# VisualComputingInstitute/diffusion-e2e-ft

Measured on AMD Instinct MI355X. Metric: images/sec (768x768, 1-step UNet fwd) full path: VAE encode + SD-v2 UNet @t=999 + VAE decode, higher is better.
Workload: dtype f16

## Files before the change

### diffusion-e2e-ft_amd/_lib.py

```python
import ctypes as C
import os

import torch

from . import build as _build

_LIB = None

F32, F16, BF16 = 0, 1, 2
_DT = {torch.float32: F32, torch.float16: F16, torch.bfloat16: BF16}


def dtype_id(dt):
    try:
        return _DT[dt]
    except KeyError:
        raise TypeError("libe2eft supports float32/float16/bfloat16, got %s" % dt)


class ConvDesc(C.Structure):
    _fields_ = [(n, C.c_int32) for n in (
        "dtype", "batch", "hin", "win", "hl", "wl", "c1", "ldx1", "c2", "ldx2", "kh", "kw", "stride", "pad_t", "pad_l",
        "hout", "wout", "cout", "ldo", "ldr", "ldw")] + [("alpha", C.c_float)]

# ... 47 lines not shown
class NormalGtDesc(C.Structure):
    _fields_ = [(n, C.c_int32) for n in ("batch", "height", "width", "raw_dtype")]


NORMAL_GT_U8, NORMAL_GT_F32 = range(2)


class DsineRgbDesc(C.Structure):
    _fields_ = [(n, C.c_int32) for n in ("batch", "height", "width", "out_layout")]


class DiffusionDesc(C.Structure):
    _fields_ = [(n, C.c_int32) for n in ("dtype", "dtype_out", "prediction", "rows", "hw", "c", "batch", "ldx0", "ldn", "ldy", "n_timesteps")]


DIFFUSION_ADD_NOISE, DIFFUSION_VELOCITY = range(2)
PREDICTION_TYPES = {"epsilon": 0, "v_prediction": 1}


RGB_HWC, RGB_CHW = range(2)
DSINE_RGB_WS_INTS = 6


OPT_PERSISTENT, OPT_PERSISTENT_GRID, OPT_NARROW_CONV, OPT_NARROW_MFMA, OPT_IGEMM_GENERAL_OPERANDS, OPT_IGEMM2_WAVES, OPT_PATCH_CONV, OPT_THIN_INPUT_CONV, OPT_FUSED_NORM, OPT_ATTN_DMA, OPT_UPCONV_PHASES, OPT_PATCH_CONV_2X2, OPT_PERSISTENT_MIN_QROUNDS, OPT_GN_APPLY_ITERS, OPT_F32_SPLIT, OPT_F32_SPLIT_ATTN, OPT_PATCH_MFMA = range(17)

_P = C.c_void_p
_I = C.c_int32
_L = C.c_int64
_F = C.c_float
_Z = C.c_size_t

SIGNATURES = {
    "e2eft_version": (_I, []),
    "e2eft_last_error": (C.c_char_p, []),
    "e2eft_build_id": (C.c_char_p, []),
    "e2eft_set_option": (_I, [_I, _I]),
    "e2eft_get_option": (_I, [_I]),
    "e2eft_conv2d_fwd": (_I, [C.POINTER(ConvDesc), _P, _P, _P, _P, _P, _P, _P, _P]),
    "e2eft_gemm": (_I, [C.POINTER(GemmDesc), _P, _P, _P, _P, _P, _P]),
    "e2eft_conv2d_fwd_gnstats": (_I, [C.POINTER(ConvDesc), _P, _P, _P, _P, _P, _P, _P, _P, _Z, C.POINTER(C.c_int32), _P]),
    "e2eft_conv2d_splitk_workspace_bytes": (_Z, [C.POINTER(ConvDesc)]),
    "e2eft_conv2d_fwd_splitk": (_I, [C.POINTER(ConvDesc), _P, _P, _P, _P, _P, _P, _P, _P, _Z, _P]),
    "e2eft_gemm_gnstats": (_I, [C.POINTER(GemmDesc), _P, _P, _P, _P, _P, _I, _P, _Z, C.POINTER(C.c_int32), _P]),
    "e2eft_groupnorm_fwd_pre": (_I, [C.POINTER(GroupNormDesc), _P, _P, _P, _P, _P, _P, _I, _P, _I, _P, _Z, _P]),
    "e2eft_groupnorm_coeff_offset": (_Z, [C.POINTER(GroupNormDesc)]),
    "e2eft_groupnorm_fwd_stats": (_I, [C.POINTER(GroupNormDesc), _P, _P, _P, _P, _I, _P, _I, _P, _Z, _P]),
    "e2eft_conv2d_fwd_normed_supported": (_I, [C.POINTER(ConvDesc)]),
    "e2eft_upconv2x_fwd_supported": (_I, [C.POINTER(ConvDesc)]),
    "e2eft_upconv2x_fwd": (_I, [C.POINTER(ConvDesc), _P, _P, _P, _P, _P, _Z, C.POINTER(C.c_int32), _P]),
    "e2eft_groupnorm_fwd_split": (_I, [C.POINTER(GroupNormDesc), _P, _P, _P, _P, _I, _P, _P, _I, _P, _Z, _P]),
    "e2eft_f32_split_weight": (_I, [_P, _L, _I, _P, _P, _P]),
    "e2eft_f32_split2_cat": (_I, [_P, _I, _I, _P, _I, _I, _L, _P, _I, _P, _P]),
    "e2eft_f32_split2": (_I, [_P, _L, _I, _I, _P, _I, _P, _P]),
    "e2eft_f32_split2_cols": (_I, [_P, _I, _I, _P, _I, _I, _L, _P, _I, _P, _P]),
    "e2eft_f32_split_wgrad_finish": (_I, [_P, _P, _P, _L, _I, _I, _P, _P, _P, _P]),
    "e2eft_conv2d_fwd_f32split_supported": (_I, [C.POINTER(ConvDesc)]),
    "e2eft_conv2d_fwd_f32split": (_I, [C.POINTER(ConvDesc), _P, _P, _P, _P, _P, _P, _P, _P, _Z, C.POINTER(C.c_int32), _P]),
    "e2eft_upconv2x_fwd_f32split_supported": (_I, [C.POINTER(ConvDesc)]),
    "e2eft_upconv2x_fwd_f32split": (_I, [C.POINTER(ConvDesc), _P, _P, _P, _P, _P, _P, _P, _Z, C.POINTER(C.c_int32), _P]),
    "e2eft_gemm_f32split_supported": (_I, [C.POINTER(GemmDesc)]),
    "e2eft_attn_f32split_supported": (_I, [C.POINTER(AttnDesc), _I]),
    "e2eft_gemm_f32split": (_I, [C.POINTER(GemmDesc), _P, _P, _P, _P, _P, _P, _P, _P]),
    "e2eft_conv2d_fwd_normed": (_I, [C.POINTER(ConvDesc), _P, _P, _P, _I, _P, _P, _P, _P, _P, _P, _Z, C.POINTER(C.c_int32), _P]),
    "e2eft_groupnorm_workspace_bytes": (_Z, [C.POINTER(GroupNormDesc)]),
    "e2eft_groupnorm_fwd": (_I, [C.POINTER(GroupNormDesc), _P, _P, _P, _P, _P, _P, _Z, _P]),
    "e2eft_layernorm_fwd": (_I, [_I, _L, _I, _I, _I, _F, _P, _P, _P, _P, _P]),
    "e2eft_geglu_fwd": (_I, [_I, _L, _I, _I, _I, _P, _P, _P]),
    "e2eft_softmax_rows": (_I, [_I, _L, _I, _L, _F, _P, _P]),
    "e2eft_softmax_rows_causal": (_I, [_I, _L, _I, _L, _F, _I, _P, _P]),
    "e2eft_attn_fwd": (_I, [C.POINTER(AttnDesc), _P, _P, _P, _P, _P]),
    "e2eft_attn_fwd_lse": (_I, [C.POINTER(AttnDesc), _P, _P, _P, _P, _P, _P]),
    "e2eft_attn512_workspace_bytes": (_Z, [C.POINTER(AttnDesc)]),
    "e2eft_attn512_fwd": (_I, [C.POINTER(AttnDesc), _P, _P, _P, _P, _P, _Z, _P]),
    "e2eft_attn_bwd_workspace_bytes": (_Z, [C.POINTER(AttnDesc)]),
    "e2eft_attn_bwd": (_I, [C.POINTER(AttnDesc), _P, _P, _P, _P, _P, _I, _P, _P, _I, _P, _I, _P, _I, _P, _Z, _P]),
    "e2eft_nchw_to_nhwc": (_I, [_I, _I, _I, _I, _I, _I, _I, _F, _F, _P, _P, _P]),
    "e2eft_nhwc_to_nchw": (_I, [_I, _I, _I, _I, _I, _I, _F, _F, _P, _P, _P]),
    "e2eft_copy_scale": (_I, [_I, _L, _I, _I, _I, _F, _F, _P, _P, _P]),
    "e2eft_add": (_I, [_I, _L, _I, _I, _I, _I, _P, _P, _P, _P]),
    "e2eft_timestep_embedding": (_I, [_I, _I, _I, _P, _P, _P]),
    "e2eft_silu": (_I, [_I, _L, _P, _P, _P]),
    "e2eft_depth_head": (_I, [_I, _I, _L, _I, _I, _P, _P, _P]),
    "e2eft_normal_head": (_I, [_I, _I, _I, _I, _I, _I, _F, _P, _P, _P]),
    "e2eft_ssi_loss_workspace_bytes": (_Z, [_I]),
    "e2eft_ssi_loss_fwd": (_I, [_I, _I, _P, _P, _P, _P, _P, _P, _Z, _P]),
    "e2eft_angular_loss_workspace_bytes": (_Z, [_I]),
    "e2eft_angular_loss_fwd": (_I, [_I, _I, _P, _P, _P, _P, _P, _Z, _P]),
    "e2eft_conv2d_dgrad": (_I, [C.POINTER(ConvDesc), _P, _I, _I, _P, _I, _P, _I, _P]),
    "e2eft_conv2d_wgrad_workspace_bytes": (_Z, [C.POINTER(ConvDesc), _I]),
# ... 138 lines not shown
```

### diffusion-e2e-ft_amd/csrc/api.hip

```cpp
#include "common.h"
#include <atomic>

namespace e2eft {

static thread_local char g_err[512] = "";

char* err_buf() { return g_err; }

int fail(int code, const char* fmt, ...) {
    va_list ap;
    va_start(ap, fmt);
    vsnprintf(g_err, sizeof(g_err), fmt, ap);
    va_end(ap);
    return code;
}

int check_launch(const char* what) {
    hipError_t e = hipGetLastError();
    if (e != hipSuccess) return fail(E2EFT_ERR_LAUNCH, "%s: launch failed: %s", what, hipGetErrorString(e));
    return E2EFT_OK;
}

static std::atomic<int> g_cus_of_device[64];
int device_cus() {
    int dev = 0;
    if (hipGetDevice(&dev) != hipSuccess || dev < 0 || dev >= 64) return 0;
    int n = g_cus_of_device[dev].load(std::memory_order_relaxed);
    if (n == 0) {
        if (hipDeviceGetAttribute(&n, hipDeviceAttributeMultiprocessorCount, dev) != hipSuccess || n < 8) return 0;
        n &= ~7;
        g_cus_of_device[dev].store(n, std::memory_order_relaxed);
    }
    return n;
}

static thread_local char g_tag[96] = "";
void tag_kernel(const char* fmt, ...) {
    va_list ap;
    va_start(ap, fmt);
    vsnprintf(g_tag, sizeof(g_tag), fmt, ap);
    va_end(ap);
}
const char* last_tag() { return g_tag; }

static std::atomic<int> g_opt[E2EFT_OPT_COUNT] = {{1}, {0}, {1}, {1}, {0}, {0}, {1}, {1}, {1}, {1}, {1}, {1}, {2}, {0}, {1}, {0}, {0}};

int option(int key) { return g_opt[key].load(std::memory_order_relaxed); }

}

extern "C" int e2eft_set_option(int32_t key, int32_t value) {
    using namespace e2eft;
    E2EFT_REQUIRE(key >= 0 && key < E2EFT_OPT_COUNT, "set_option: unknown key %d", key);
    bool ok = value == 0 || value == 1;
    if (key == E2EFT_OPT_PERSISTENT_GRID) ok = value == 0 || (value >= 8 && value % 8 == 0 && value <= 4096);
    if (key == E2EFT_OPT_IGEMM2_WAVES) ok = value == 0 || value == 4 || value == 8;
    if (key == E2EFT_OPT_PERSISTENT_MIN_QROUNDS) ok = value >= 1 && value <= 64;
    if (key == E2EFT_OPT_GN_APPLY_ITERS) ok = value >= 0 && value <= 16;
    if (key == E2EFT_OPT_PATCH_MFMA) ok = value >= 0 && value <= 2;
    E2EFT_REQUIRE(ok, "set_option: value %d out of range for key %d", value, key);
    g_opt[key].store(value, std::memory_order_relaxed);
    return E2EFT_OK;
}
extern "C" int e2eft_get_option(int32_t key) { return key >= 0 && key < E2EFT_OPT_COUNT ? e2eft::option(key) : -1; }

extern "C" const char* e2eft_debug_last_kernel(void) { return e2eft::last_tag(); }

extern "C" int e2eft_version(void) { return E2EFT_VERSION; }
// ... 7 lines not shown
```

### diffusion-e2e-ft_amd/csrc/gfx950.h

```cpp
#pragma once
#include "common.h"
#include <type_traits>

namespace e2eft {

template <int V> using IConst = std::integral_constant<int, V>;

template <typename T> struct Mma32x32x16;
template <> struct Mma32x32x16<f16> {
    __device__ static __forceinline__ floatx16 run(const u32x4& a, const u32x4& b, floatx16 c) {
        return __builtin_amdgcn_mfma_f32_32x32x16_f16(__builtin_bit_cast(half8, a), __builtin_bit_cast(half8, b), c, 0, 0, 0);
    }
};
template <> struct Mma32x32x16<bf16> {
    __device__ static __forceinline__ floatx16 run(const u32x4& a, const u32x4& b, floatx16 c) {
        return __builtin_amdgcn_mfma_f32_32x32x16_bf16(__builtin_bit_cast(bhalf8, a), __builtin_bit_cast(bhalf8, b), c, 0, 0, 0);
    }
};

template <typename T> struct Mma16x16x32;
template <> struct Mma16x16x32<f16> {
    __device__ static __forceinline__ floatx4 run(const u32x4& a, const u32x4& b, floatx4 c) {
        return __builtin_amdgcn_mfma_f32_16x16x32_f16(__builtin_bit_cast(half8, a), __builtin_bit_cast(half8, b), c, 0, 0, 0);
    }
};
template <> struct Mma16x16x32<bf16> {
    __device__ static __forceinline__ floatx4 run(const u32x4& a, const u32x4& b, floatx4 c) {
        return __builtin_amdgcn_mfma_f32_16x16x32_bf16(__builtin_bit_cast(bhalf8, a), __builtin_bit_cast(bhalf8, b), c, 0, 0, 0);
    }
};

typedef float float2v __attribute__((ext_vector_type(2)));
typedef __bf16 bhalf2v __attribute__((ext_vector_type(2)));
template <typename T> __device__ __forceinline__ uint32_t pack2(float lo, float hi);
template <> __device__ __forceinline__ uint32_t pack2<f16>(float lo, float hi) {
    const float2v f = {lo, hi};
    return __builtin_bit_cast(uint32_t, __builtin_convertvector(f, half2v));
}
template <> __device__ __forceinline__ uint32_t pack2<bf16>(float lo, float hi) {
    const float2v f = {lo, hi};
    return __builtin_bit_cast(uint32_t, __builtin_convertvector(f, bhalf2v));
}

__device__ __forceinline__ int fast_div(int n, int d) {
    int q = (int)((float)n * __builtin_amdgcn_rcpf((float)d));
    const int r = n - q * d;
    if (r < 0) --q;
    else if (r >= d) ++q;
    return q;
}

typedef __attribute__((address_space(3))) void* lds_ptr_t;

__device__ __forceinline__ u32x2 lds_read_tr16(const char* p) {
    typedef short short4v __attribute__((ext_vector_type(4)));
    return __builtin_bit_cast(u32x2, __builtin_amdgcn_ds_read_tr16_b64_v4i16((__attribute__((address_space(3))) short4v*)p));
}

constexpr unsigned int SRD_RECORDS = 0xE0000000u;
constexpr unsigned int SRD_OOB = 0xF0000000u;
constexpr long SRD_SPAN_MAX = 0xD0000000L, SRD_TILE_MAX = 0x40000000L;
__device__ __forceinline__ __amdgpu_buffer_rsrc_t whole_range_rsrc(const void* base) {
    return __builtin_amdgcn_make_buffer_rsrc((void*)base, 0, SRD_RECORDS, 0x00020000);
}
// ... 25 lines not shown
```

### diffusion-e2e-ft_amd/csrc/narrow.hip

```cpp
#include "gfx950.h"

namespace e2eft {

constexpr int NR_T = 16;
constexpr int NR_H = NR_T + 2;
constexpr int NR_CH = 64;
constexpr int NR_PIX = NR_CH * 2 + 16;
constexpr int NR_CO = 4;

typedef _Float16 h2 __attribute__((ext_vector_type(2)));
typedef __bf16 b2 __attribute__((ext_vector_type(2)));
typedef short s2 __attribute__((ext_vector_type(2)));

template <typename T> __device__ __forceinline__ float dot2(unsigned a, unsigned b, float c);
template <> __device__ __forceinline__ float dot2<f16>(unsigned a, unsigned b, float c) {
    return __builtin_amdgcn_fdot2(__builtin_bit_cast(h2, a), __builtin_bit_cast(h2, b), c, false);
}
template <> __device__ __forceinline__ float dot2<bf16>(unsigned a, unsigned b, float c) {
    return __builtin_amdgcn_fdot2_f32_bf16(__builtin_bit_cast(s2, a), __builtin_bit_cast(s2, b), c, false);
}
template <typename T> __device__ __forceinline__ float dot16(const u32x4& a, const u32x4& b, float s) {
    if constexpr (sizeof(T) == 4) {
        const floatx4 fa = __builtin_bit_cast(floatx4, a), fb = __builtin_bit_cast(floatx4, b);
        s = fmaf(fa[0], fb[0], s); s = fmaf(fa[1], fb[1], s); s = fmaf(fa[2], fb[2], s); s = fmaf(fa[3], fb[3], s);
    } else {
        s = dot2<T>(a[0], b[0], s); s = dot2<T>(a[1], b[1], s); s = dot2<T>(a[2], b[2], s); s = dot2<T>(a[3], b[3], s);
    }
    return s;
}

struct NarrowParams {
    const void* x;
    const void* w;
    const void* bias;
    void* out;
    int H, W, cin, ldx, ldw, cout, ldo, tiles_x, tiles_y;
    float alpha;
    const float* nrm_ad;
    const void* nrm_beta;
    int nrm_silu;
};

typedef const __attribute__((address_space(4))) u32x4* cptr_t;

template <typename T, int CO>
__global__ __launch_bounds__(256) void conv3x3_narrow_kernel(const NarrowParams p, const T* __restrict__ wg) {
    __shared__ __attribute__((aligned(16))) char halo[NR_H * NR_H * NR_PIX];
    const int tid = threadIdx.x;
    const int tx = tid & 15, ty = tid >> 4;
    const int tile = blockIdx.x;
    const int oy0 = (tile / p.tiles_x) * NR_T, ox0 = (tile % p.tiles_x) * NR_T;
    const T* xb = (const T*)p.x + (long)blockIdx.y * p.H * p.W * p.ldx;
// ... 205 lines not shown
```

### diffusion-e2e-ft_amd/csrc/norm.hip

```cpp
#include "common.h"

namespace e2eft {

struct Triple {
    float n, mean, m2;
};
__device__ __forceinline__ Triple merge(const Triple& A, const Triple& B) {
    if (B.n == 0.f) return A;
    if (A.n == 0.f) return B;
    Triple r;
    r.n = A.n + B.n;
    const float delta = B.mean - A.mean;
    const float f = B.n / r.n;
    r.mean = A.mean + delta * f;
    r.m2 = A.m2 + B.m2 + delta * delta * A.n * f;
    return r;
}

struct GnGeom {
    int batch, hw, c1, ldx1, c2, ldx2, C;
    int nchunks, cpb, nchb, pl;
    int nslabs, slab;
};

// ... 562 lines not shown
    const float mean = wave_sum(sum) / (float)c;
    float sq = 0.f;
#pragma unroll
    for (int i = 0; i < MAXI; ++i) {
        const int ch = lane + 64 * i;
        if (ch < nchunks) {
#pragma unroll
            for (int e = 0; e < EPC; ++e) { const float dd = v[i][e] - mean; sq += dd * dd; }
        }
    }
    const float rstd = rsqrtf(wave_sum(sq) / (float)c + eps);
#pragma unroll
    for (int i = 0; i < MAXI; ++i) {
        const int ch = lane + 64 * i;
        if (ch < nchunks) {
            Vec16<T> ga = ld16(gamma + ch * EPC), be = ld16(beta + ch * EPC), o;
#pragma unroll
            for (int e = 0; e < EPC; ++e) o.e[e] = from_f<T>((v[i][e] - mean) * rstd * to_f(ga.e[e]) + to_f(be.e[e]));
            st16(y + row * ldy + ch * EPC, o);
        }
    }
}

template <typename T>
__global__ __launch_bounds__(256) void softmax_rows_kernel(int ntot, long lds, float scale, T* __restrict__ s, int causal_nq) {
    constexpr int EPC = 16 / (int)sizeof(T);
    __shared__ float red[8];
    T* row = s + (long)blockIdx.x * lds;
    const int tid = threadIdx.x, lane = tid & 63, wave = tid >> 6;
    const int n = causal_nq > 0 ? min(ntot, (int)(blockIdx.x % (unsigned)causal_nq) + 1) : ntot;
    const int nfull = n / EPC;
    const float sc = scale * 1.4426950408889634f;
    float mx = -INFINITY;
    for (int ch = tid; ch < nfull; ch += 256) {
        Vec16<T> v = ld16(row + ch * EPC);
#pragma unroll
        for (int e = 0; e < EPC; ++e) mx = fmaxf(mx, to_f(v.e[e]));
    }
    for (int j = nfull * EPC + tid; j < n; j += 256) mx = fmaxf(mx, to_f(row[j]));
    mx = wave_max(mx);
    if (lane == 0) red[wave] = mx;
    __syncthreads();
    mx = fmaxf(fmaxf(red[0], red[1]), fmaxf(red[2], red[3]));
    const float mb = mx * sc;
    float sum = 0.f;
    for (int ch = tid; ch < nfull; ch += 256) {
// ... 258 lines not shown
}

extern "C" int e2eft_layernorm_fwd(int32_t dtype, int64_t rows, int32_t c, int32_t ldx, int32_t ldy, float eps,
                                   const void* x, const void* gamma, const void* beta, void* y, void* stream) {
    E2EFT_REQUIRE(x && gamma && beta && y, "layernorm: null pointer");
    E2EFT_REQUIRE(dtype >= 0 && dtype <= 2, "layernorm: bad dtype");
    const int epc = 16 / (int)dtype_size(dtype);
    E2EFT_REQUIRE(rows > 0 && c > 0 && c % epc == 0 && ldx >= c && ldy >= c && ldx % epc == 0 && ldy % epc == 0, "layernorm: shape c=%d ldx=%d ldy=%d", c, ldx, ldy);
    const int nchunks = c / epc;
    E2EFT_REQUIRE(nchunks <= 64 * 8, "layernorm: c=%d too large", c);
    const long nblk = (rows + 3) / 4;
    E2EFT_REQUIRE(nblk < 2147483647L, "layernorm: too many rows");
    hipStream_t s = (hipStream_t)stream;
    const int iters = (nchunks + 63) / 64;
#define LN_LAUNCH(T, MAXI) hipLaunchKernelGGL((layernorm_kernel<T, MAXI>), dim3((unsigned)nblk), dim3(256), 0, s, (long)rows, c, ldx, ldy, eps, (const T*)x, (const T*)gamma, (const T*)beta, (T*)y)
    E2EFT_DISPATCH_DTYPE(dtype, T, {
        if (iters <= 1) LN_LAUNCH(T, 1);
        else if (iters <= 2) LN_LAUNCH(T, 2);
        else if (iters <= 4) LN_LAUNCH(T, 4);
        else LN_LAUNCH(T, 8);
    });
#undef LN_LAUNCH
    return check_launch("layernorm");
}

extern "C" int e2eft_softmax_rows(int32_t dtype, int64_t rows, int32_t n, int64_t lds, float scale, void* sbuf, void* stream) {
    E2EFT_REQUIRE(sbuf, "softmax: null pointer");
    E2EFT_REQUIRE(dtype >= 0 && dtype <= 2, "softmax: bad dtype");
    const int epc = 16 / (int)dtype_size(dtype);
    E2EFT_REQUIRE(rows > 0 && rows < 2147483647L && n > 0 && lds >= (n + epc - 1) / epc * epc && lds % epc == 0, "softmax: shape n=%d lds=%ld", n, (long)lds);
    E2EFT_REQUIRE(scale > 0.f, "softmax: scale must be positive");
    hipStream_t s = (hipStream_t)stream;
    E2EFT_DISPATCH_DTYPE(dtype, T, hipLaunchKernelGGL((softmax_rows_kernel<T>), dim3((unsigned)rows), dim3(256), 0, s, n, (long)lds, scale, (T*)sbuf, 0));
    return check_launch("softmax_rows");
}

extern "C" int e2eft_softmax_rows_causal(int32_t dtype, int64_t rows, int32_t n, int64_t lds, float scale, int32_t nq, void* sbuf, void* stream) {
    E2EFT_REQUIRE(sbuf, "softmax_causal: null pointer");
    E2EFT_REQUIRE(dtype >= 0 && dtype <= 2, "softmax_causal: bad dtype");
    const int epc = 16 / (int)dtype_size(dtype);
    E2EFT_REQUIRE(rows > 0 && rows < 2147483647L && n > 0 && lds >= (n + epc - 1) / epc * epc && lds % epc == 0, "softmax_causal: shape n=%d lds=%ld", n, (long)lds);
    E2EFT_REQUIRE(nq > 0 && nq <= n && rows % nq == 0, "softmax_causal: nq=%d must divide rows and be <= n (self-attention)", nq);
    E2EFT_REQUIRE(scale > 0.f, "softmax_causal: scale must be positive");
    hipStream_t s = (hipStream_t)stream;
    E2EFT_DISPATCH_DTYPE(dtype, T, hipLaunchKernelGGL((softmax_rows_kernel<T>), dim3((unsigned)rows), dim3(256), 0, s, n, (long)lds, scale, (T*)sbuf, (int)nq));
    return check_launch("softmax_rows_causal");
// ... 119 lines not shown
```

### diffusion-e2e-ft_amd/modules.py

```python

import torch
from torch import nn

from . import ops
from . import autograd as F


_cached = F.cached


def packed_conv_weight(conv):
    return F.packed_conv_weight(conv, conv.weight.dtype)


def conv_nhwc(conv, x, x2=None, up_to=None, rowadd=None, residual=None, alpha=1.0, pad=None, out=None, gn_stats=True, norm=None):
    assert out is None
    return F.conv(conv, x, x2=x2, up_to=up_to, rowadd=rowadd, residual=residual, alpha=alpha, pad=pad, gn_stats=gn_stats, norm=norm)


def checkpointed(enabled, fn, *args):
    if enabled and torch.is_grad_enabled() and any(isinstance(a, torch.Tensor) and a.requires_grad for a in args):
        from torch.utils.checkpoint import checkpoint
        return checkpoint(fn, *args, use_reentrant=False)
    return fn(*args)
# ... 177 lines not shown
    def __init__(self, query_dim, heads, cross_attention_dim=None, bias=False, joint=False):
        super().__init__()
        self.heads = heads
        self.scale = (query_dim // heads) ** -0.5
        self.joint = joint
        kv = cross_attention_dim or query_dim
        self.to_q = Linear(query_dim, query_dim, bias=bias)
        self.to_k = Linear(kv, query_dim, bias=bias)
        self.to_v = Linear(kv, query_dim, bias=bias)
        self.to_out = nn.ModuleList([Linear(query_dim, query_dim), nn.Dropout(0.0)])

    def forward(self, x, ctx=None, residual=None):
        B, N, C = x.shape
        d = C // self.heads
        out = self.to_out[0]
        kv_pre = None
        shared_src = None
        if isinstance(ctx, CtxCond):
            kv_pre = ctx.kv.get(id(self))
            shared_src = ctx.src if ctx.shared else None
            ctx = ctx.ctx
        if F.needs_grad(x, ctx, self.to_q.weight, self.to_k.weight, self.to_v.weight, out.weight):
            return out(self._forward_train(x, ctx), residual=residual)
        if (CROSS_ATTN_FOLD and shared_src is not None and shared_src.shape[1] == 2 and not self.joint and self.to_q.bias is None and self.to_k.bias is None
                and self.to_v.bias is None and self.heads <= 64):
            return self._folded(x, shared_src, residual)
        fused = F.fused_attention_ok(x.dtype, d)
        dt = x.dtype
        if fused:
            if ctx is None:
                qkv = F.linear(x, (self.to_q.weight, self.to_k.weight, self.to_v.weight), owner=self, name="wqkv")
                q, k, v = qkv[..., :C], qkv[..., C:2 * C], qkv[..., 2 * C:]
            else:
                q = self.to_q(x)
                kv = kv_pre
                if kv is None or torch.is_grad_enabled():
                    kv = F.linear(ctx, (self.to_k.weight, self.to_v.weight), owner=self, name="wkv")
                k, v = kv[..., :C], kv[..., C:]
            a = ops.attention(q, k, v, self.heads, self.scale, kv_nseg=2 if self.joint else 1, kv_bmod=B // 2 if self.joint else B)
        else:
            src = x if ctx is None else ctx
            cw = lambda lin: F._cat_weight(lin, "w", (lin.weight,), dt, lin.weight.shape[1])
            a = attention_unfused(x, src, cw(self.to_q), F._vec(self.to_q.bias, dt), cw(self.to_k), F._vec(self.to_k.bias, dt), cw(self.to_v),
                                  F._vec(self.to_v.bias, dt), self.heads, self.scale, joint=self.joint)
        return out(a, residual=residual)

    def _fold(self, src, dt):
        out = self.to_out[0]
        ws = [w for w in (self.to_q.weight, self.to_k.weight, self.to_v.weight, out.weight, out.bias) if w is not None]
        key = (src.data_ptr(), src._version, tuple(src.shape), str(src.device), dt, F._key(*ws))
        hit = self.__dict__.get("_fold_cache")
        if hit is not None and hit[0] == key:
            return hit[1]
        with torch.no_grad():
            h, C = self.heads, self.to_q.weight.shape[0]
            d = C // h
            f32 = lambda w: w.detach().float().contiguous()
            wq, wk, wv, wo = f32(self.to_q.weight), f32(self.to_k.weight), f32(self.to_v.weight), f32(out.weight)
            c32 = f32(src[0])
            k = ops.gemm(c32, wk)
            v = ops.gemm(c32, wv)
            ar = torch.arange(h, device=k.device)
            Mk = torch.zeros((h, h, d), dtype=torch.float32, device=k.device)
            Mv = torch.zeros((h, h, d), dtype=torch.float32, device=k.device)
            Mk[ar, ar] = (k[0] - k[1]).view(h, d) * self.scale
            Mv[ar, ar] = (v[0] - v[1]).view(h, d)
            G = ops.gemm(Mk.view(h, C), wq.t().contiguous())
            delta = ops.gemm(Mv.view(h, C), wo)
# ... 42 lines not shown
class FeedForward(nn.Module):

    def __init__(self, dim):
        super().__init__()
        self.net = nn.ModuleList([GEGLU(dim, 4 * dim), nn.Dropout(0.0), Linear(4 * dim, dim)])

    def forward(self, x, residual=None):
        return self.net[2](self.net[0](x), residual=residual)


class BasicTransformerBlock(nn.Module):

    def __init__(self, dim, heads, cross_attention_dim, joint=False):
        super().__init__()
        self.norm1 = LayerNorm(dim, eps=1e-5)
        self.attn1 = Attention(dim, heads, joint=joint)
        self.norm2 = LayerNorm(dim, eps=1e-5)
        self.attn2 = Attention(dim, heads, cross_attention_dim=cross_attention_dim)
        self.norm3 = LayerNorm(dim, eps=1e-5)
        self.ff = FeedForward(dim)

    def forward(self, h, ctx):
        h = self.attn1(self.norm1(h), None, residual=h)
        h = self.attn2(self.norm2(h), ctx, residual=h)
        return self.ff(self.norm3(h), residual=h)


class Transformer2DModel(nn.Module):

    def __init__(self, channels, heads, cross_attention_dim, groups=32, joint=False):
        super().__init__()
        self.norm = GroupNorm(groups, channels, eps=1e-6, affine=True)
        self.proj_in = Linear(channels, channels)
        self.transformer_blocks = nn.ModuleList([BasicTransformerBlock(channels, heads, cross_attention_dim, joint=joint)])
        self.proj_out = Linear(channels, channels)

    def nhwc(self, x, ctx):
        B, H, W, C = x.shape
        h, x = self.norm.nhwc(x, split=True)
        h = self.proj_in(h.view(B, H * W, C))
        for blk in self.transformer_blocks:
            h = blk(h, ctx)
        out = self.proj_out(h, residual=x.reshape(B, H * W, C), gn_rows_per_image=H * W)
        res = out.view(B, H, W, C)
        st = getattr(out, "_e2eft_gn", None)
        if st is not None:
            res._e2eft_gn = st
# ... 39 lines not shown
```

### diffusion-e2e-ft_amd/ops.py

```python
import ctypes as C
from types import SimpleNamespace

import torch

from . import _lib
from ._lib import ConvDesc, GemmDesc, GroupNormDesc, AttnDesc, check, dtype_id


class KernelTimer:

    def __init__(self, only=None):
        self.rec = {}
        self.only = only

    def add(self, name, start, end, flops, nbytes, label=None, launches=1, flops_nominal=None):
        self.rec.setdefault(name, []).append((start, end, flops, nbytes, label, launches, flops if flops_nominal is None else flops_nominal))

    def summary(self):
        torch.cuda.synchronize()
        out = {}
        for name, lst in self.rec.items():
            ms = sum(r[0].elapsed_time(r[1]) for r in lst)
            out[name] = dict(launches=sum(r[5] for r in lst), ms=ms, flops=float(sum(r[2] for r in lst)), bytes=float(sum(r[3] for r in lst)),
                             flops_nominal=float(sum(r[6] for r in lst)))
# ... 658 lines not shown

def groupnorm_stats(x, gamma, groups, eps):
    _check_cuda(x, gamma)
    B, H, W, c1 = x.shape
    d = _gn_desc(x, None, groups, eps, False, c1)
    ws, nbytes = _gn_workspace(d, x.device, "groupnorm_stats")
    s1 = getattr(x, "_e2eft_gn", None) if GN_STATS_ENABLED else None
    lib = _lib.load()
    with _timed("groupnorm_stats", 0.0, 0.0, label="gn stats B%d %dx%d C%d" % (B, H, W, c1)):
        check(lib.e2eft_groupnorm_fwd_stats(C.byref(d), _ptr(x), C.c_void_p(0), _ptr(gamma), *_gn_stats_args(s1), C.c_void_p(0), 0, _ptr(ws), nbytes, _stream()))
    return ws, ws.data_ptr() + lib.e2eft_groupnorm_coeff_offset(C.byref(d))


def layernorm(x, gamma, beta, eps, out=None):
    _check_cuda(x, gamma, beta, out)
    Cc = x.shape[-1]
    a = x.reshape(-1, Cc) if x.is_contiguous() else _as_rows(x)
    if out is None:
        out = torch.empty(x.shape, dtype=x.dtype, device=x.device)
    o = out.reshape(-1, Cc) if out.is_contiguous() else _as_rows(out)
    assert gamma.dtype == x.dtype and beta.dtype == x.dtype
    check(_lib.load().e2eft_layernorm_fwd(dtype_id(x.dtype), a.shape[0], Cc, _rows_ld(a), _rows_ld(o), eps, _ptr(a), _ptr(gamma),
                                         _ptr(beta), _ptr(o), _stream()))
    return out


def geglu(h, out=None):
    _check_cuda(h, out)
    c2 = h.shape[-1]
    c = c2 // 2
    a = h.reshape(-1, c2) if h.is_contiguous() else _as_rows(h)
    if out is None:
        out = torch.empty((*h.shape[:-1], c), dtype=h.dtype, device=h.device)
    o = out.reshape(-1, c) if out.is_contiguous() else _as_rows(out)
    check(_lib.load().e2eft_geglu_fwd(dtype_id(h.dtype), a.shape[0], c, _rows_ld(a), _rows_ld(o), _ptr(a), _ptr(o), _stream()))
    return out


def softmax_rows_(s, n, scale, causal_nq=0):
    _check_cuda(s)
    assert s.dim() == 2 and s.is_contiguous()
    if causal_nq:
        check(_lib.load().e2eft_softmax_rows_causal(dtype_id(s.dtype), s.shape[0], n, s.shape[1], scale, causal_nq, _ptr(s), _stream()))
    else:
        check(_lib.load().e2eft_softmax_rows(dtype_id(s.dtype), s.shape[0], n, s.shape[1], scale, _ptr(s), _stream()))
    return s
# ... 1082 lines not shown
```

### include/e2eft.h

```cpp
#ifndef E2EFT_H
#define E2EFT_H

#include <stddef.h>
#include <stdint.h>

#ifdef __cplusplus
extern "C" {
#endif
#pragma GCC visibility push(default)

#define E2EFT_VERSION 119

enum {
    E2EFT_OK = 0,
    E2EFT_ERR_BAD_ARG = 1,
    E2EFT_ERR_WORKSPACE = 2,
    E2EFT_ERR_LAUNCH = 3,
    E2EFT_ERR_UNSUPPORTED = 4,
};

enum { E2EFT_F32 = 0, E2EFT_F16 = 1, E2EFT_BF16 = 2 };

int e2eft_version(void);
const char* e2eft_last_error(void);
const char* e2eft_build_id(void);

enum {
    E2EFT_OPT_PERSISTENT = 0,
    E2EFT_OPT_PERSISTENT_GRID = 1,
    E2EFT_OPT_NARROW_CONV = 2,
    E2EFT_OPT_NARROW_MFMA = 3,
    E2EFT_OPT_IGEMM_GENERAL_OPERANDS = 4,
    E2EFT_OPT_IGEMM2_WAVES = 5,
    E2EFT_OPT_PATCH_CONV = 6,
    E2EFT_OPT_THIN_INPUT_CONV = 7,
    E2EFT_OPT_FUSED_NORM = 8,
    E2EFT_OPT_ATTN_DMA = 9,
    E2EFT_OPT_UPCONV_PHASES = 10,
    E2EFT_OPT_PATCH_CONV_2X2 = 11,
    E2EFT_OPT_PERSISTENT_MIN_QROUNDS = 12,
    E2EFT_OPT_GN_APPLY_ITERS = 13,
    E2EFT_OPT_F32_SPLIT = 14,
    E2EFT_OPT_F32_SPLIT_ATTN = 15,
    E2EFT_OPT_PATCH_MFMA = 16,
    E2EFT_OPT_COUNT = 17
};
int e2eft_set_option(int32_t key, int32_t value);
int e2eft_get_option(int32_t key);

typedef struct E2eftConvDesc {
    int32_t dtype;
    int32_t batch, hin, win, hl, wl;
    int32_t c1, ldx1;
    int32_t c2, ldx2;
    int32_t kh, kw, stride;
    int32_t pad_t, pad_l;
    int32_t hout, wout;
    int32_t cout, ldo;
    int32_t ldr;
    int32_t ldw;
    float alpha;
} E2eftConvDesc;

int e2eft_conv2d_fwd(const E2eftConvDesc* d, const void* x1, const void* x2, const void* w,
                     const void* bias ,
                     const void* rowadd ,
                     const void* residual , void* out, void* stream);

// ... 51 lines not shown
    int32_t c1, ldx1, c2, ldx2;
    int32_t groups;
    int32_t ldy;
    int32_t silu;
    float eps;
} E2eftGroupNormDesc;

size_t e2eft_groupnorm_workspace_bytes(const E2eftGroupNormDesc* d);
int e2eft_groupnorm_fwd(const E2eftGroupNormDesc* d, const void* x1, const void* x2, const void* gamma,
                        const void* beta, void* y, void* workspace, size_t ws_bytes, void* stream);

int e2eft_groupnorm_fwd_split(const E2eftGroupNormDesc* d, const float* x, const float* gamma, const float* beta, void* planes, int32_t ldp, float* scale,
                              const float* partial1, int32_t nslabs1, void* workspace, size_t ws_bytes, void* stream);

int e2eft_groupnorm_fwd_pre(const E2eftGroupNormDesc* d, const void* x1, const void* x2, const void* gamma,
                            const void* beta, void* y, const float* partial1, int32_t nslabs1, const float* partial2,
                            int32_t nslabs2, void* workspace, size_t ws_bytes, void* stream);
size_t e2eft_groupnorm_coeff_offset(const E2eftGroupNormDesc* d);
int e2eft_groupnorm_fwd_stats(const E2eftGroupNormDesc* d, const void* x1, const void* x2, const void* gamma, const float* partial1,
                              int32_t nslabs1, const float* partial2, int32_t nslabs2, void* workspace, size_t ws_bytes, void* stream);

int e2eft_layernorm_fwd(int32_t dtype, int64_t rows, int32_t c, int32_t ldx, int32_t ldy, float eps,
                        const void* x, const void* gamma, const void* beta, void* y, void* stream);

int e2eft_geglu_fwd(int32_t dtype, int64_t rows, int32_t c, int32_t ldh, int32_t ldy, const void* h, void* y,
                    void* stream);

int e2eft_softmax_rows(int32_t dtype, int64_t rows, int32_t n, int64_t lds, float scale, void* s, void* stream);
int e2eft_softmax_rows_causal(int32_t dtype, int64_t rows, int32_t n, int64_t lds, float scale, int32_t nq, void* s, void* stream);

typedef struct E2eftAttnDesc {
    int32_t dtype;
    int32_t batch, heads, nq, nk_seg;
    int32_t kv_nseg, kv_bmod;
    int32_t ldq, ldk, ldv, ldo;
    float scale;
} E2eftAttnDesc;

int e2eft_attn_fwd(const E2eftAttnDesc* d, const void* q, const void* k, const void* v, void* out, void* stream);
int e2eft_attn_fwd_lse(const E2eftAttnDesc* d, const void* q, const void* k, const void* v, void* out, float* lse, void* stream);
int32_t e2eft_attn_f32split_supported(const E2eftAttnDesc* d, int32_t backward);
size_t e2eft_attn512_workspace_bytes(const E2eftAttnDesc* d);
int e2eft_attn512_fwd(const E2eftAttnDesc* d, const void* q, const void* k, const void* v, void* out, void* workspace, size_t ws_bytes,
                      void* stream);
size_t e2eft_conv2d_wgrad_workspace_bytes(const E2eftConvDesc* d, int32_t lddy);
int e2eft_conv2d_wgrad(const E2eftConvDesc* d, const void* dy, int32_t lddy, const void* x1, const void* x2, float* partial, size_t partial_bytes,
// ... 214 lines not shown
```

Baseline: 92.60.

## Fuse LayerNorm with folded two-token cross-attention into one kernel

Adds a kernel that computes LayerNorm per row, projects the normalized row onto per-head fold vectors G, applies a sigmoid (two-key softmax), mixes the precomputed Dt rows and c0, and adds the residual, all in one pass. The transformer block now uses it for attn2 whenever the shared-context fold applies. This removes the separate LayerNorm output write/read and the separate folded-attention kernels, in exchange for a large LDS footprint (up to 144KB) and a capped persistent grid. The shared dot2/dot16 helpers move into a common header.

```diff
diff --git a/diffusion-e2e-ft_amd/_lib.py b/diffusion-e2e-ft_amd/_lib.py
--- a/diffusion-e2e-ft_amd/_lib.py
+++ b/diffusion-e2e-ft_amd/_lib.py
@@ -93,7 +93,7 @@
 DSINE_RGB_WS_INTS = 6
 
 
-OPT_PERSISTENT, OPT_PERSISTENT_GRID, OPT_NARROW_CONV, OPT_NARROW_MFMA, OPT_IGEMM_GENERAL_OPERANDS, OPT_IGEMM2_WAVES, OPT_PATCH_CONV, OPT_THIN_INPUT_CONV, OPT_FUSED_NORM, OPT_ATTN_DMA, OPT_UPCONV_PHASES, OPT_PATCH_CONV_2X2, OPT_PERSISTENT_MIN_QROUNDS, OPT_GN_APPLY_ITERS, OPT_F32_SPLIT, OPT_F32_SPLIT_ATTN, OPT_PATCH_MFMA = range(17)
+OPT_PERSISTENT, OPT_PERSISTENT_GRID, OPT_NARROW_CONV, OPT_NARROW_MFMA, OPT_IGEMM_GENERAL_OPERANDS, OPT_IGEMM2_WAVES, OPT_PATCH_CONV, OPT_THIN_INPUT_CONV, OPT_FUSED_NORM, OPT_ATTN_DMA, OPT_UPCONV_PHASES, OPT_PATCH_CONV_2X2, OPT_PERSISTENT_MIN_QROUNDS, OPT_GN_APPLY_ITERS, OPT_F32_SPLIT, OPT_F32_SPLIT_ATTN, OPT_PATCH_MFMA, OPT_LN_CROSS_FOLD = range(18)
 
 _P = C.c_void_p
 _I = C.c_int32
@@ -136,6 +136,7 @@
     "e2eft_groupnorm_workspace_bytes": (_Z, [C.POINTER(GroupNormDesc)]),
     "e2eft_groupnorm_fwd": (_I, [C.POINTER(GroupNormDesc), _P, _P, _P, _P, _P, _P, _Z, _P]),
     "e2eft_layernorm_fwd": (_I, [_I, _L, _I, _I, _I, _F, _P, _P, _P, _P, _P]),
+    "e2eft_ln_cross_fold": (_I, [_I, _L, _I, _I, _I, _I, _F, _P, _P, _P, _P, _P, _P, _P, _P]),
     "e2eft_geglu_fwd": (_I, [_I, _L, _I, _I, _I, _P, _P, _P]),
     "e2eft_softmax_rows": (_I, [_I, _L, _I, _L, _F, _P, _P]),
     "e2eft_softmax_rows_causal": (_I, [_I, _L, _I, _L, _F, _I, _P, _P]),
diff --git a/diffusion-e2e-ft_amd/csrc/api.hip b/diffusion-e2e-ft_amd/csrc/api.hip
--- a/diffusion-e2e-ft_amd/csrc/api.hip
+++ b/diffusion-e2e-ft_amd/csrc/api.hip
@@ -43,7 +43,7 @@
 }
 const char* last_tag() { return g_tag; }
 
-static std::atomic<int> g_opt[E2EFT_OPT_COUNT] = {{1}, {0}, {1}, {1}, {0}, {0}, {1}, {1}, {1}, {1}, {1}, {1}, {2}, {0}, {1}, {0}, {0}};
+static std::atomic<int> g_opt[E2EFT_OPT_COUNT] = {{1}, {0}, {1}, {1}, {0}, {0}, {1}, {1}, {1}, {1}, {1}, {1}, {2}, {0}, {1}, {0}, {0}, {1}};
 
 int option(int key) { return g_opt[key].load(std::memory_order_relaxed); }
 
diff --git a/diffusion-e2e-ft_amd/csrc/gfx950.h b/diffusion-e2e-ft_amd/csrc/gfx950.h
--- a/diffusion-e2e-ft_amd/csrc/gfx950.h
+++ b/diffusion-e2e-ft_amd/csrc/gfx950.h
@@ -40,6 +40,24 @@
 template <> __device__ __forceinline__ uint32_t pack2<bf16>(float lo, float hi) {
     const float2v f = {lo, hi};
     return __builtin_bit_cast(uint32_t, __builtin_convertvector(f, bhalf2v));
+}
+
+typedef short short2v __attribute__((ext_vector_type(2)));
+template <typename T> __device__ __forceinline__ float dot2(unsigned a, unsigned b, float c);
+template <> __device__ __forceinline__ float dot2<f16>(unsigned a, unsigned b, float c) {
+    return __builtin_amdgcn_fdot2(__builtin_bit_cast(half2v, a), __builtin_bit_cast(half2v, b), c, false);
+}
+template <> __device__ __forceinline__ float dot2<bf16>(unsigned a, unsigned b, float c) {
+    return __builtin_amdgcn_fdot2_f32_bf16(__builtin_bit_cast(short2v, a), __builtin_bit_cast(short2v, b), c, false);
+}
+template <typename T> __device__ __forceinline__ float dot16(const u32x4& a, const u32x4& b, float s) {
+    if constexpr (sizeof(T) == 4) {
+        const floatx4 fa = __builtin_bit_cast(floatx4, a), fb = __builtin_bit_cast(floatx4, b);
+        s = fmaf(fa[0], fb[0], s); s = fmaf(fa[1], fb[1], s); s = fmaf(fa[2], fb[2], s); s = fmaf(fa[3], fb[3], s);
+    } else {
+        s = dot2<T>(a[0], b[0], s); s = dot2<T>(a[1], b[1], s); s = dot2<T>(a[2], b[2], s); s = dot2<T>(a[3], b[3], s);
+    }
+    return s;
 }
 
 __device__ __forceinline__ int fast_div(int n, int d) {
diff --git a/diffusion-e2e-ft_amd/csrc/narrow.hip b/diffusion-e2e-ft_amd/csrc/narrow.hip
--- a/diffusion-e2e-ft_amd/csrc/narrow.hip
+++ b/diffusion-e2e-ft_amd/csrc/narrow.hip
@@ -7,27 +7,6 @@
 constexpr int NR_CH = 64;
 constexpr int NR_PIX = NR_CH * 2 + 16;
 constexpr int NR_CO = 4;
-
-typedef _Float16 h2 __attribute__((ext_vector_type(2)));
-typedef __bf16 b2 __attribute__((ext_vector_type(2)));
-typedef short s2 __attribute__((ext_vector_type(2)));
-
-template <typename T> __device__ __forceinline__ float dot2(unsigned a, unsigned b, float c);
-template <> __device__ __forceinline__ float dot2<f16>(unsigned a, unsigned b, float c) {
-    return __builtin_amdgcn_fdot2(__builtin_bit_cast(h2, a), __builtin_bit_cast(h2, b), c, false);
-}
-template <> __device__ __forceinline__ float dot2<bf16>(unsigned a, unsigned b, float c) {
-    return __builtin_amdgcn_fdot2_f32_bf16(__builtin_bit_cast(s2, a), __builtin_bit_cast(s2, b), c, false);
-}
-template <typename T> __device__ __forceinline__ float dot16(const u32x4& a, const u32x4& b, float s) {
-    if constexpr (sizeof(T) == 4) {
-        const floatx4 fa = __builtin_bit_cast(floatx4, a), fb = __builtin_bit_cast(floatx4, b);
-        s = fmaf(fa[0], fb[0], s); s = fmaf(fa[1], fb[1], s); s = fmaf(fa[2], fb[2], s); s = fmaf(fa[3], fb[3], s);
-    } else {
-        s = dot2<T>(a[0], b[0], s); s = dot2<T>(a[1], b[1], s); s = dot2<T>(a[2], b[2], s); s = dot2<T>(a[3], b[3], s);
-    }
-    return s;
-}
 
 struct NarrowParams {
     const void* x;
diff --git a/diffusion-e2e-ft_amd/csrc/norm.hip b/diffusion-e2e-ft_amd/csrc/norm.hip
--- a/diffusion-e2e-ft_amd/csrc/norm.hip
+++ b/diffusion-e2e-ft_amd/csrc/norm.hip
@@ -1,4 +1,4 @@
-#include "common.h"
+#include "gfx950.h"
 
 namespace e2eft {
 
@@ -608,6 +608,180 @@
     }
 }
 
+
+template <int N, int O = 32> __device__ __forceinline__ void wave_reduce_scatter(float (&a)[N], const int lane) {
+    if constexpr (O >= 1) {
+        if constexpr (N > 1) {
+            constexpr int H = N / 2;
+            const bool up = (lane & O) != 0;
+            float k[H];
+#pragma unroll
+            for (int t = 0; t < H; ++t) {
+                if constexpr (O == 32 || O == 16) {
+                    const unsigned lo = __builtin_bit_cast(unsigned, a[t]), hi = __builtin_bit_cast(unsigned, a[t + H]);
+                    const auto sw = O == 32 ? __builtin_amdgcn_permlane32_swap(lo, hi, false, false) : __builtin_amdgcn_permlane16_swap(lo, hi, false, false);
+                    k[t] = __builtin_bit_cast(float, (unsigned)sw[0]) + __builtin_bit_cast(float, (unsigned)sw[1]);
+                } else {
+                    const float send = up ? a[t] : a[t + H], keep = up ? a[t + H] : a[t];
+                    k[t] = keep + __shfl_xor(send, O, 64);
+                }
+            }
+            wave_reduce_scatter<H, O / 2>(k, lane);
+            a[0] = k[0];
+        } else {
+            a[0] += __shfl_xor(a[0], O, 64);
+            wave_reduce_scatter<1, O / 2>(a, lane);
+        }
+    }
+}
+
+constexpr int LCF_THREADS = 512, LCF_WAVES = LCF_THREADS / 64;
+
+template <typename T, int MAXI, int NH, int LDSB, int HEADS>
+__global__ __launch_bounds__(LCF_THREADS) void ln_cross_fold_kernel(long rows, int c, int heads_rt, int hp_rt, int ldx, int ldo, float eps, const T* __restrict__ x,
+                                                                    const T* __restrict__ gamma, const T* __restrict__ beta, const T* __restrict__ G,
+                                                                    const T* __restrict__ Dt, const T* __restrict__ c0, T* __restrict__ out) {
+    static_assert(sizeof(T) == 2, "16-bit tensors");
+    constexpr int EPC = 8, SH = 6 - (NH == 8 ? 3 : NH == 16 ? 4 : 5);
+    static_assert(NH == 8 || NH == 16 || NH == 32, "head slots");
+    __shared__ __attribute__((aligned(16))) char smem[LDSB];
+    const int tid = threadIdx.x, lane = tid & 63, wave = tid >> 6;
+    static_assert(HEADS <= NH, "head slots");
+    const int heads = HEADS ? HEADS : heads_rt, hp = HEADS ? (HEADS + 7) / 8 * 8 : hp_rt;
+    const int nchunks = c / EPC, hq = hp / EPC, dpitch = nchunks | 1;
+    u32x4* sG = reinterpret_cast<u32x4*>(smem);
+    u32x4* sD = sG + heads * nchunks;
+    u32x4* sV = sD + EPC * hq * dpitch;
+    const long stride = (long)gridDim.x * LCF_WAVES;
+    long row = (long)blockIdx.x * LCF_WAVES + wave;
+    auto load_row = [&](const long r, u32x4 (&raw)[MAXI]) {
+#pragma unroll
+        for (int i = 0; i < MAXI; ++i) {
+            const int ch = lane + 64 * i;
+            raw[i] = u32x4{0u, 0u, 0u, 0u};
+            if (r < rows && ch < nchunks) raw[i] = *reinterpret_cast<const u32x4*>(x + r * ldx + ch * EPC);
+        }
+    };
+    float v[MAXI][EPC];
+    auto unpack = [&](const u32x4 (&raw)[MAXI]) {
+#pragma unroll
+        for (int i = 0; i < MAXI; ++i) {
+            Vec16<T> t;
+            t.raw = raw[i];
+#pragma unroll
+            for (int e = 0; e < EPC; ++e) {
+                v[i][e] = to_f(t.e[e]);
+                asm volatile("" : "+v"(v[i][e]));
+            }
+        }
+    };
+    u32x4 raw[MAXI];
+    load_row(row, raw);
+    for (int u = tid; u < heads * nchunks; u += LCF_THREADS) sG[u] = reinterpret_cast<const u32x4*>(G)[u];
+    {
+        for (int u = tid; u < c * hq; u += LCF_THREADS) {
+            const int cc = u / hq, q = u - cc * hq;
+            sD[((cc & 7) * hq + q) * dpitch + (cc >> 3)] = reinterpret_cast<const u32x4*>(Dt)[u];
+        }
+        for (int u = tid; u < nchunks; u += LCF_THREADS) {
+            sV[u] = reinterpret_cast<const u32x4*>(gamma)[u];
+            sV[nchunks + u] = reinterpret_cast<const u32x4*>(beta)[u];
+            sV[2 * nchunks + u] = reinterpret_cast<const u32x4*>(c0)[u];
+        }
+    }
+    __syncthreads();
+    unpack(raw);
+    while (row < rows) {
+        load_row(row + stride, raw);
+        float sum = 0.f;
+#pragma unroll
+        for (int i = 0; i < MAXI; ++i) {
+#pragma unroll
+            for (int e = 0; e < EPC; ++e) sum += v[i][e];
+        }
+        const float mean = wave_sum(sum) / (float)c;
+        float sq = 0.f;
+#pragma unroll
+        for (int i = 0; i < MAXI; ++i) {
+            if (lane + 64 * i < nchunks) {
+#pragma unroll
+                for (int e = 0; e < EPC; ++e) { const float dd = v[i][e] - mean; sq += dd * dd; }
+            }
+        }
+        const float rstd = rsqrtf(wave_sum(sq) / (float)c + eps);
+        float part[NH];
+#pragma unroll
+        for (int j = 0; j < NH; ++j) part[j] = 0.f;
+#pragma unroll
+        for (int i = 0; i < MAXI; ++i) {
+            const int ch = lane + 64 * i;
+            if (ch < nchunks) {
+                Vec16<T> y;
+                float ga[EPC], be[EPC];
+                {
+                    Vec16<T> gv, bv;
+                    gv.raw = sV[ch];
+                    bv.raw = sV[nchunks + ch];
+#pragma unroll
+                    for (int e = 0; e < EPC; ++e) { ga[e] = to_f(gv.e[e]); be[e] = to_f(bv.e[e]); }
+                }
+#pragma unroll
+                for (int e = 0; e < EPC; ++e) y.e[e] = from_f<T>((v[i][e] - mean) * rstd * ga[e] + be[e]);
+#pragma unroll
+                for (int j = 0; j < NH; ++j)
+                    if (j < heads) part[j] = dot16<T>(y.raw, sG[j * nchunks + ch], part[j]);
+            }
+        }
+        wave_reduce_scatter<NH>(part, lane);
+        const float pl = __builtin_amdgcn_rcpf(1.0f + __expf(-part[0]));
+        float p[NH];
+        Vec16<T> o[MAXI];
+#pragma unroll
+        for (int j = 0; j < NH; ++j) p[j] = __builtin_bit_cast(float, __builtin_amdgcn_readlane(__builtin_bit_cast(int, pl), j << SH));
+#pragma unroll
+        for (int i = 0; i < MAXI; ++i) {
+            const int ch = lane + 64 * i;
+            if (ch < nchunks) {
+                {
+                    Vec16<T> cv;
+                    cv.raw = sV[2 * nchunks + ch];
+#pragma unroll
+                    for (int e = 0; e < EPC; ++e) {
+                        float acc = 0.f;
+#pragma unroll
+                        for (int q = 0; q < NH / EPC; ++q) {
+                            if (q * EPC < heads) {
+                                Vec16<T> d;
+                                d.raw = sD[(e * hq + q) * dpitch + ch];
+#pragma unroll
+                                for (int k = 0; k < EPC; ++k)
+                                    if (q * EPC + k < heads) acc = fmaf(p[q * EPC + k], to_f(d.e[k]), acc);
+                            }
+                        }
+                        o[i].e[e] = from_f<T>(acc + to_f(cv.e[e]) + v[i][e]);
+                    }
+                }
+            }
+        }
+        unpack(raw);
+#pragma unroll
+        for (int i = 0; i < MAXI; ++i) {
+            const int ch = lane + 64 * i;
+            if (ch < nchunks) st16(out + row * ldo + ch * EPC, o[i]);
+        }
+        row += stride;
+    }
+}
+
+static size_t lcf_lds_bytes(int c, int heads, int hp) { return ((size_t)heads * (c / 8) + (size_t)hp * ((c / 8) | 1) + 3 * (size_t)(c / 8)) * 16; }
+static int lcf_class(int c, int heads, int hp) {
+    const size_t need = lcf_lds_bytes(c, heads, hp);
+    if (c <= 512 && heads <= 8 && need <= 20 * 1024) return 1;
+    if (c <= 1024 && heads <= 16 && need <= 72 * 1024) return 2;
+    if (c <= 1536 && heads <= 32 && need <= 144 * 1024) return 3;
+    return 0;
+}
+
 template <typename T>
 __global__ __launch_bounds__(256) void softmax_rows_kernel(int ntot, long lds, float scale, T* __restrict__ s, int causal_nq) {
     constexpr int EPC = 16 / (int)sizeof(T);
@@ -912,6 +1086,41 @@
     });
 #undef LN_LAUNCH
     return check_launch("layernorm");
+}
+
+extern "C" int e2eft_ln_cross_fold(int32_t dtype, int64_t rows, int32_t c, int32_t heads, int32_t ldx, int32_t ldo, float eps, const void* x,
+                                   const void* gamma, const void* beta, const void* g, const void* delta_t, const void* c0, void* out, void* stream) {
+    E2EFT_REQUIRE(x && gamma && beta && g && delta_t && c0 && out, "ln_cross_fold: null pointer");
+    E2EFT_REQUIRE(dtype == E2EFT_F16 || dtype == E2EFT_BF16, "ln_cross_fold: 16-bit tensors only (dtype %d)", (int)dtype);
+    E2EFT_REQUIRE(rows > 0 && c > 0 && c % 8 == 0 && heads >= 1 && ldx >= c && ldo >= c && ldx % 8 == 0 && ldo % 8 == 0,
+                  "ln_cross_fold: shape c=%d heads=%d ldx=%d ldo=%d", c, heads, ldx, ldo);
+    E2EFT_REQUIRE(al16(x) && al16(gamma) && al16(beta) && al16(g) && al16(delta_t) && al16(c0) && al16(out), "ln_cross_fold: pointers must be 16-byte aligned");
+    const int hp = (heads + 7) / 8 * 8;
+    const int cls = lcf_class(c, heads, hp);
+    if (cls == 0 || !option(E2EFT_OPT_LN_CROSS_FOLD))
+        return fail(E2EFT_ERR_UNSUPPORTED, "ln_cross_fold: c=%d heads=%d is outside the kernel's three classes, or E2EFT_OPT_LN_CROSS_FOLD is 0", c, heads);
+    const int cus = device_cus();
+    E2EFT_REQUIRE(cus > 0, "ln_cross_fold: no device");
+    const long want = (rows + LCF_WAVES - 1) / LCF_WAVES, cap = (long)cus * (cls == 1 ? 4 : cls == 2 ? 2 : 1);
+    const dim3 grid((unsigned)(want < cap ? want : cap));
+    hipStream_t s = (hipStream_t)stream;
+#define LCF_LAUNCH(T, MAXI, NH, KB, HEADS)                                                                                                           \
+    hipLaunchKernelGGL((ln_cross_fold_kernel<T, MAXI, NH, KB * 1024, HEADS>), grid, dim3(LCF_THREADS), 0, s, (long)rows, c, heads, hp, ldx, ldo, eps, (const T*)x, \
+                       (const T*)gamma, (const T*)beta, (const T*)g, (const T*)delta_t, (const T*)c0, (T*)out)
+#define LCF_CLASS(T)                             \
+    do {                                         \
+        if (cls == 1 && heads == 5) LCF_LAUNCH(T, 1, 8, 20, 5);        \
+        else if (cls == 1) LCF_LAUNCH(T, 1, 8, 20, 0);                 \
+        else if (cls == 2 && heads == 10) LCF_LAUNCH(T, 2, 16, 72, 10); \
+        else if (cls == 2) LCF_LAUNCH(T, 2, 16, 72, 0);                \
+        else if (heads == 20) LCF_LAUNCH(T, 3, 32, 144, 20);           \
+        else LCF_LAUNCH(T, 3, 32, 144, 0);                             \
+    } while (0)
+    if (dtype == E2EFT_F16) LCF_CLASS(f16);
+    else LCF_CLASS(bf16);
+#undef LCF_CLASS
+#undef LCF_LAUNCH
+    return check_launch("ln_cross_fold");
 }
 
 extern "C" int e2eft_softmax_rows(int32_t dtype, int64_t rows, int32_t n, int64_t lds, float scale, void* sbuf, void* stream) {
diff --git a/diffusion-e2e-ft_amd/modules.py b/diffusion-e2e-ft_amd/modules.py
--- a/diffusion-e2e-ft_amd/modules.py
+++ b/diffusion-e2e-ft_amd/modules.py
@@ -223,8 +223,7 @@
             ctx = ctx.ctx
         if F.needs_grad(x, ctx, self.to_q.weight, self.to_k.weight, self.to_v.weight, out.weight):
             return out(self._forward_train(x, ctx), residual=residual)
-        if (CROSS_ATTN_FOLD and shared_src is not None and shared_src.shape[1] == 2 and not self.joint and self.to_q.bias is None and self.to_k.bias is None
-                and self.to_v.bias is None and self.heads <= 64):
+        if self._foldable(shared_src):
             return self._folded(x, shared_src, residual)
         fused = F.fused_attention_ok(x.dtype, d)
         dt = x.dtype
@@ -245,6 +244,19 @@
             a = attention_unfused(x, src, cw(self.to_q), F._vec(self.to_q.bias, dt), cw(self.to_k), F._vec(self.to_k.bias, dt), cw(self.to_v),
                                   F._vec(self.to_v.bias, dt), self.heads, self.scale, joint=self.joint)
         return out(a, residual=residual)
+
+    def _foldable(self, shared_src):
+        return (CROSS_ATTN_FOLD and shared_src is not None and shared_src.shape[1] == 2 and not self.joint and self.to_q.bias is None and self.to_k.bias is None
+                and self.to_v.bias is None and self.heads <= 64)
+
+    def normed_fold(self, norm, h, ctx):
+        src = ctx.src if isinstance(ctx, CtxCond) and ctx.shared else None
+        out = self.to_out[0]
+        if (not self._foldable(src) or not ops.ln_cross_fold_ok(h.dtype, h.shape[-1], self.heads)
+                or F.needs_grad(h, ctx.ctx, norm.weight, norm.bias, self.to_q.weight, self.to_k.weight, self.to_v.weight, out.weight)):
+            return None
+        G, Dt, c0 = self._fold(src, h.dtype)
+        return ops.ln_cross_fold(h, F._vec(norm.weight, h.dtype), F._vec(norm.bias, h.dtype), norm.eps, G, Dt, c0, self.heads)
 
     def _fold(self, src, dt):
         out = self.to_out[0]
@@ -333,7 +345,8 @@
 
     def forward(self, h, ctx):
         h = self.attn1(self.norm1(h), None, residual=h)
-        h = self.attn2(self.norm2(h), ctx, residual=h)
+        fused = self.attn2.normed_fold(self.norm2, h, ctx)
+        h = fused if fused is not None else self.attn2(self.norm2(h), ctx, residual=h)
         return self.ff(self.norm3(h), residual=h)
 
 
diff --git a/diffusion-e2e-ft_amd/ops.py b/diffusion-e2e-ft_amd/ops.py
--- a/diffusion-e2e-ft_amd/ops.py
+++ b/diffusion-e2e-ft_amd/ops.py
@@ -704,6 +704,32 @@
     assert gamma.dtype == x.dtype and beta.dtype == x.dtype
     check(_lib.load().e2eft_layernorm_fwd(dtype_id(x.dtype), a.shape[0], Cc, _rows_ld(a), _rows_ld(o), eps, _ptr(a), _ptr(gamma),
                                          _ptr(beta), _ptr(o), _stream()))
+    return out
+
+
+def ln_cross_fold_ok(dtype, c, heads):
+    if dtype not in (torch.float16, torch.bfloat16) or c % 8 or heads < 1:
+        return False
+    units = heads * (c // 8) + round_up(heads, 8) * ((c // 8) | 1) + 3 * (c // 8)
+    fits = any(c <= cm and heads <= hm and units * 16 <= kb * 1024 for cm, hm, kb in ((512, 8, 20), (1024, 16, 72), (1536, 32, 144)))
+    return fits and _lib.load().e2eft_get_option(_lib.OPT_LN_CROSS_FOLD) == 1
+
+
+def ln_cross_fold(x, gamma, beta, eps, G, Dt, c0, heads, out=None):
+    _check_cuda(x, gamma, beta, G, Dt, c0, out)
+    Cc = x.shape[-1]
+    a = x.reshape(-1, Cc) if x.is_contiguous() else _as_rows(x)
+    if out is None:
+        out = torch.empty(x.shape, dtype=x.dtype, device=x.device)
+    o = out.reshape(-1, Cc) if out.is_contiguous() else _as_rows(out)
+    hp = round_up(heads, 8)
+    assert all(t.dtype == x.dtype and t.is_contiguous() for t in (gamma, beta, G, Dt, c0))
+    assert G.shape[0] >= heads and G.shape[1] == Cc and tuple(Dt.shape) == (Cc, hp) and gamma.numel() == beta.numel() == c0.numel() == Cc
+    rows = a.shape[0]
+    es = x.element_size()
+    with _timed("ln_cross_fold", 4.0 * rows * Cc * heads, 2.0 * rows * Cc * es, label="ln_cross_fold M%d C%d heads%d" % (rows, Cc, heads)):
+        check(_lib.load().e2eft_ln_cross_fold(dtype_id(x.dtype), rows, Cc, heads, _rows_ld(a), _rows_ld(o), eps, _ptr(a), _ptr(gamma), _ptr(beta), _ptr(G),
+                                             _ptr(Dt), _ptr(c0), _ptr(o), _stream()))
     return out
 
 
diff --git a/include/e2eft.h b/include/e2eft.h
--- a/include/e2eft.h
+++ b/include/e2eft.h
@@ -43,7 +43,8 @@
     E2EFT_OPT_F32_SPLIT = 14,
     E2EFT_OPT_F32_SPLIT_ATTN = 15,
     E2EFT_OPT_PATCH_MFMA = 16,
-    E2EFT_OPT_COUNT = 17
+    E2EFT_OPT_LN_CROSS_FOLD = 17,
+    E2EFT_OPT_COUNT = 18
 };
 int e2eft_set_option(int32_t key, int32_t value);
 int e2eft_get_option(int32_t key);
@@ -141,6 +142,9 @@
 
 int e2eft_layernorm_fwd(int32_t dtype, int64_t rows, int32_t c, int32_t ldx, int32_t ldy, float eps,
                         const void* x, const void* gamma, const void* beta, void* y, void* stream);
+
+int e2eft_ln_cross_fold(int32_t dtype, int64_t rows, int32_t c, int32_t heads, int32_t ldx, int32_t ldo, float eps, const void* x,
+                        const void* gamma, const void* beta, const void* g, const void* delta_t, const void* c0, void* out, void* stream);
 
 int e2eft_geglu_fwd(int32_t dtype, int64_t rows, int32_t c, int32_t ldh, int32_t ldy, const void* h, void* y,
                     void* stream);
```

New measurement: 93.21 (median of 6 runs). About the same (+0.7%).
